# abhishekiitm/CSED_514_Project_Distributed_Training_using_PyTorch

Hardware: AMD Instinct MI355X
Metric: MNIST epoch time (s) + images/sec at 1/2/4/8 MI355X (DDP) (higher is better)
Workload: dtype bf16

## Files before the change

csrc/kernels/lenet_dev.h:

```cpp
#pragma once
#include <hip/hip_runtime.h>
#include <stdint.h>

#include "common.h"

namespace csed {

typedef short s16x8 __attribute__((ext_vector_type(8)));
typedef short s16x4 __attribute__((ext_vector_type(4)));
typedef unsigned short u16x4 __attribute__((ext_vector_type(4)));
typedef __attribute__((address_space(3))) s16x4 lds_s16x4;
typedef __attribute__((address_space(3))) void lds_void;
typedef __attribute__((address_space(1))) void glb_void;

template <typename T>
__device__ __forceinline__ unsigned short h16(float v) { return bits_of<T>((T)v); }
template <typename T>
__device__ __forceinline__ float f16v(unsigned short b) { return (float)of_bits<T>(b); }

__device__ __forceinline__ s16x4 lds_read_tr16(const unsigned short* p) {
  return __builtin_amdgcn_ds_read_tr16_b64_v4i16((lds_s16x4*)(p));
}


__device__ __forceinline__ int opaque(int x) {
  asm("" : "+v"(x));
  return x;
}

__device__ __forceinline__ void lds_barrier() { asm volatile("s_waitcnt lgkmcnt(0)\n\ts_barrier" ::: "memory"); }

template <int OFF>
__device__ __forceinline__ uint32_t lds_u16(const unsigned short* p) {
  uint32_t v;
  asm volatile("ds_read_u16 %0, %1 offset:%2" : "=v"(v) : "v"((uint32_t)reinterpret_cast<uintptr_t>(p)), "i"(OFF * 2));
  return v;
}
__device__ __forceinline__ void lds_wait8(uint32_t (&v)[8]) {
  asm volatile("s_waitcnt lgkmcnt(0)"
               : "+v"(v[0]), "+v"(v[1]), "+v"(v[2]), "+v"(v[3]), "+v"(v[4]), "+v"(v[5]), "+v"(v[6]), "+v"(v[7]));
}

__device__ __forceinline__ void store16_wt(const void* base, int byte_off, float4 v) {
  typedef unsigned int u32x4v_ __attribute__((ext_vector_type(4)));
  __builtin_amdgcn_raw_buffer_store_b128(__builtin_bit_cast(u32x4v_, v),
                                         __builtin_amdgcn_make_buffer_rsrc(const_cast<void*>(base), (short)0,
                                                                           0x7fffffff, 0x00020000),
                                         byte_off, 0, 16);
}

}
```

csrc/kernels/lenet_fused.hip:

```cpp
#include <algorithm>
#include <cmath>
#include <cstdlib>
#include <type_traits>

#include "comm/ipc_allreduce.h"
#include "common.h"
#include "dispatch.h"
#include "kernels/lenet_dev.h"
#include "kernels/lenet_images.h"
#include "kernels/lenet_layout.h"

namespace csed {

namespace lenet {
constexpr int LD_DC2 = 72, LD_DC1 = 592;
constexpr int LD_P1 = 148;
constexpr int NT = 1024, NW = 16;

constexpr int S_W2C = 0;
constexpr int S_W2D = (I_W2D - I_W2C) * 2;
constexpr int S_F1 = (I_F1 - I_W2C) * 2;
constexpr int WIMG_LDS_U4 = (I_END - I_W2C) / 8;
constexpr int S_X = (I_END - I_W2C) * 2;
constexpr int S_P1 = S_X + 800 * 2;
constexpr int S_I1 = S_P1 + 10 * LD_P1 * 2;
constexpr int S_P2 = S_I1 + (10 * LD_P1 + 15) / 16 * 16;
constexpr int S_I2 = S_P2 + 320 * 2;
constexpr int S_P1H = S_I2 + 320;
constexpr int S_DC2 = S_P1H + 12 * P1H_RP * 2;
constexpr int S_DC2H = S_DC2 + 32 * LD_DC2 * 2;
constexpr int S_DC1 = S_DC2H + 16 * DC2H_RP * 2;
constexpr int S_COFF = S_DC1 + 16 * LD_DC1 * 2;
constexpr int S_DOFF = S_COFF + 4 * 16 * 2;
constexpr int S_DZ1B = S_DOFF + 4 * 24 * 2;
constexpr int S_F = S_DZ1B + 64 * 2;
constexpr int F_D2S = 0, F_D1S = 32, F_H = 96, F_LOGIT = 160, F_PAR = 176, F_RED = 768, F_END = 2816;
constexpr int P_C1B = 0, P_C2B = 10, P_F1B = 30, P_F2B = 80, P_F2W = 90;
constexpr int S_W1C = S_F + F_END * 4;
constexpr int S_LABEL = S_W1C + 16 * 32 * 2;
constexpr int S_DBG = S_LABEL + 16;
constexpr int S_C1T = S_DBG + 32 * 8;
constexpr int S_C1H = S_C1T + 1024 * 8;
constexpr int S_XC = S_C1H + 1024 * 8;
constexpr int XC_LD = 800;
constexpr int S_CONSTB = S_XC + 3 * XC_LD * 2;
constexpr int S_TOTAL = S_CONSTB + 16 * 2;
static_assert(S_W2D % 16 == 0 && S_F1 % 16 == 0 && S_X % 16 == 0 && S_P1 % 16 == 0 && S_I1 % 16 == 0, "align");
static_assert(S_P2 % 16 == 0 && S_I2 % 16 == 0 && S_P1H % 16 == 0 && S_DC2 % 16 == 0 && S_DC2H % 16 == 0, "align");
static_assert(S_DC1 % 16 == 0 && S_COFF % 16 == 0 && S_DOFF % 16 == 0 && S_DZ1B % 16 == 0, "align");
static_assert(S_F % 16 == 0 && (F_RED * 4) % 16 == 0 && S_TOTAL <= 160 * 1024, "lds");
static_assert(WIMG_LDS_U4 % 256 == 0, "whole LDS-DMA rounds over waves 0-3");
static_assert(C2_KS * 32 <= LD_W2C && 25 * C2_ICP <= C2_KS * 32, "conv2 K");
static_assert(25 * DG_OCP <= DG_KS * 32, "dgrad K");
}

using namespace lenet;


constexpr int DBG_W = 32;
#define WSTAMP(w, i)                                                          \
  do {                                                                        \
    if (a.dbg && wave == (w) && lane == 0) DBGS[(i)] = __builtin_amdgcn_s_memtime(); \
  } while (0)
#define STAMP(i)                                                              \
  do {                                                                        \
    if (a.dbg && tid == 0 && s == (nsamp > 1 ? 1 : 0)) DBGS[(i)] = __builtin_amdgcn_s_memtime(); \
  } while (0)

__device__ const int64_t kZeroWord = 0;

__device__ __forceinline__ int64_t readlane64(int64_t v, int l) {
  const int lo = __builtin_amdgcn_readlane((int)(v & 0xffffffff), l);
  const int hi = __builtin_amdgcn_readlane((int)(v >> 32), l);
  return ((int64_t)hi << 32) | (uint32_t)lo;
}

template <typename T>
__device__ __forceinline__ void dgrad_store(unsigned short* DC1, int ci, int mm, float v, int bi) {
  const int ih = mm / 12, iw = mm - ih * 12;
  uint32_t* d = reinterpret_cast<uint32_t*>(DC1 + ci * LD_DC1 + (2 * ih) * 24 + 2 * iw);
  const uint32_t hv = h16<T>(v);
  d[0] = bi == 0 ? hv : (bi == 1 ? hv << 16 : 0u);
  d[12] = bi == 2 ? hv : (bi == 3 ? hv << 16 : 0u);
}

template <typename T>
__device__ __forceinline__ void dgrad_out(unsigned short* DC1, const unsigned short* P1, const uint8_t* I1,
                                          int ci, int mm, float v) {
  const int pi = ci * LD_P1 + mm;
  dgrad_store<T>(DC1, ci, mm, f16v<T>(P1[pi]) > 0.f ? v : 0.f, I1[pi]);
}

struct C1Tab {
  unsigned short v[NT][8];
};
constexpr C1Tab make_c1tab() {
  C1Tab t{};
  for (int tt = 0; tt < NT; ++tt) {
    const int tw = tt >> 6, tl16 = tt & 15, tkq = (tt & 63) >> 4;
    for (int it = 0; it < 3; ++it) {
      const int mt = (tw + it * NW) < 35 ? tw + it * NW : 35;
      const int m = mt * 16 + tl16;
      const int p = m >> 2, q = m & 3;
      t.v[tt][it] = (unsigned short)((2 * (p / 12) + (q >> 1)) * 28 + 2 * (p % 12) + (q & 1));
      const int w = mt * 4 + tkq;
      t.v[tt][4 + it] = (unsigned short)((w / 12) * P1H_RP + (w % 12) * LD_P1H);
    }
  }
  return t;
}
__constant__ C1Tab kC1Tab = make_c1tab();

constexpr int UP_C = 16, UP_S = 32, UP_MAXL = 8, UP_NT = UP_C * UP_S;

struct SplitNeed { uint32_t m[4]; };
__host__ __device__ constexpr SplitNeed split_need_table() {
  SplitNeed r{};
  for (int part = 0; part < 4; ++part) {
    uint32_t need = 0;
    for (int ts = 0; ts < (part == 0 ? 3 : 2); ++ts) {
      const int t = part + 4 * ts, py0 = (16 * t) / 12, py1 = (16 * t + 15) / 12;
      const int ps0 = (48 * py0) / 32, ps1 = (48 * (py1 + 1) - 1) / 32;
      need |= ((2u << ps1) - 1) & ~((1u << ps0) - 1);
    }
    r.m[part] = need;
  }
  return r;
}
__device__ constexpr SplitNeed kSplitNeed = split_need_table();

template <typename T, bool TRAIN, bool STAGED, int KS = 1>
__global__ void __launch_bounds__(NT, 1) lenet_train_kernel(LenetTrainArgs a, int write_logp, float* logp_out) {
  static_assert(KS == 1 || (KS == SPLIT_K && STAGED && TRAIN), "split step: staged training only");
  const uint64_t t_entry = __builtin_amdgcn_s_memtime();
  struct TrainKargs { LenetTrainArgs a; int write_logp; float* logp_out; };
// ... 78 lines not shown
  const bool stage_next = TRAIN && STAGED && a.stage_next;
  int64_t nrow = 0;
  uint32_t px_next = 0;
  int64_t lab_next = 0;
  auto conv1_tables = [&](int tt) {
    const int tw = tt >> 6, tl16 = tt & 15, tkq = (tt & 63) >> 4;
    u16x4 xo = {0, 0, 0, 0}, ho = {0, 0, 0, 0};
#pragma unroll
    for (int it = 0; it < 3; ++it) {
      const int mt = min(tw + it * NW, 35);
      const int m = mt * 16 + tl16;
      const int p = m >> 2, q = m & 3;
      xo[it] = (unsigned short)((2 * (p / 12) + (q >> 1)) * 28 + 2 * (p % 12) + (q & 1));
      const int w = mt * 4 + tkq;
      ho[it] = (unsigned short)((w / 12) * P1H_RP + (w % 12) * LD_P1H);
    }
    C1T[tt] = xo;
    C1H[tt] = ho;
  };
  if (wave < 4) {
    lds_barrier();
    constexpr int DMA_NT = 256;
    static_assert(WIMG_LDS_U4 % DMA_NT == 0, "whole LDS-DMA rounds over waves 0-3");
    const uint4* src = reinterpret_cast<const uint4*>(a.wimg + I_W2C);
#pragma unroll
    for (int u = 0; u < WIMG_LDS_U4 / DMA_NT; ++u)
      __builtin_amdgcn_global_load_lds((glb_void*)(const_cast<uint4*>(src + u * DMA_NT + tid)),
                                       (lds_void*)(wsm + S_W2C + (u * DMA_NT + wave * 64) * 16), 16, 0, 0);
    if (a.dbg && lane == 0) DBGS[(wave == 0 ? 10 : 17 + wave)] = __builtin_amdgcn_s_memtime();
  } else if (wave < 8) {
    const int t = tid - 256;
    if (a.dbg && t == 0) DBGS[17] = __builtin_amdgcn_s_memtime();
    int off0 = O_F2W - 90;
    off0 = t < 90 ? O_F2B - 80 : off0;
    off0 = t < 80 ? O_F1B - 30 : off0;
    off0 = t < 30 ? O_C2B - 10 : off0;
    off0 = t < 10 ? O_C1B : off0;
    float pv[3];
    pv[0] = a.params[off0 + t];
    pv[1] = a.params[O_F2W - 90 + 256 + t];
    pv[2] = a.params[O_F2W - 90 + min(512 + t, 589)];
    const uint4 w1 = reinterpret_cast<const uint4*>(a.wimg + I_W1C)[t & 63];
    uint32_t px0 = 0;
    int lab0 = 0;
    if (STAGED) {
      px0 = reinterpret_cast<const uint32_t*>(a.xstage + (int64_t)g * 784)[min(t, 195)];
      lab0 = (int)a.lstage[g];
    }
    if (KS == 1 && stage_next) {
      pbase = ((gptr64)curp)[opaque(0)] * (int64_t)a.B + b0;
      nrow = a.perm[min(pbase + a.B, a.perm_len - 1) + opaque(0)];
    }
    const uint64_t t_bar4 = __builtin_amdgcn_s_memtime();
    lds_barrier();
    if (t < 64) reinterpret_cast<uint4*>(W1Cs)[t] = w1;
#pragma unroll
    for (int j = 0; j < 3; ++j)
      if (t + j * 256 < 590) PAR[t + j * 256] = pv[j];
    if (STAGED) {
      if (t < 196) {
        u16x4 o;
#pragma unroll
        for (int j = 0; j < 4; ++j)
          o[j] = h16<T>(((float)((px0 >> (8 * j)) & 255u) * (1.f / 255.f) - a.mean) * inv_std);
        put_x(t, o);
      }
      if (t == 0) LABEL[0] = lab0;
    }
    if (a.dbg && t == 0) {
      DBGS[16] = __builtin_amdgcn_s_memtime();
      DBGS[15] = t_bar4;
    }
    asm volatile("" ::"v"(pv[0]), "v"(pv[1]), "v"(pv[2]), "v"(w1.x), "v"(w1.y), "v"(w1.z), "v"(w1.w), "v"(px0),
                 "v"(lab0));
  } else {
    int64_t cur = 0;
    if (STAGED) {
      rng_ctr = (uint64_t)((gptr64)rngp)[opaque(0)];
      if (KS > 1) cur = ((gptr64)curp)[opaque(0)];
    }
    const int t8 = tid - 512;
    const int tq = t8 < 64 ? t8 >> 4 : min(t8 - 64, 95) / 24;
    const int tks = t8 < 64 ? t8 & 15 : min(t8 - 64, 95) - 24 * tq;
    const int kg = t8 < 64 ? (int)kC2Order.fwd[min(4 * tks + tq, 49)] : (int)kDgOrder.fwd[min(4 * tks + tq, 74)];
    lds_barrier();
    if (t8 < 64) {
      const int tap = kg >> 1;
      COFF[t8] = (short)((tap / 5) * P1H_RP + (tap % 5) * LD_P1H + (kg & 1) * 8);
    } else if (t8 < 160) {
      const int tap = kg / 3, ocg = kg - 3 * tap;
      DOFF[t8 - 64] = (short)((tap / 5) * DC2H_RP + (tap % 5) * DG_OCP + ocg * 8);
    }
    if (!STAGED) {
      conv1_tables(tid - 512);
      conv1_tables(tid);
    }
    if (tid - 512 < 16) CONSTB[tid - 512] = tid - 512 < 8 ? (unsigned short)0 : h16<T>(1.f);
    if (STAGED) {
      if (KS > 1) pbase = cur * (int64_t)a.B + b0;
      const int tz = tid - 512;
      zero_p1h(tz);
      if (tz < 70) dropout_scales(tz, b0);
      asm volatile("" ::"v"(rng_ctr), "v"(pbase));
    }
  }
  if (!STAGED && nsamp > 0) {
    const int64_t row0 = perm_at(0);
    lab = (int)a.labels[row0];
    px = reinterpret_cast<const uint32_t*>(a.images + row0 * 784)[min(tid, 195)];
    rowv = perm_at(min(lane, nsamp - 1));
  }
  if (a.dbg && tid == 0) DBGS[13] = __builtin_amdgcn_s_memtime();
  int kwb[1];
  {
    const int k = min(wave * 16 + l16, 249), ic = k / 25, r = k % 25;
    kwb[0] = ic * LD_P1 + (r / 5) * 12 + (r % 5);
  }
  const int kc1 = (wave & 1) * 16 + l16;
  const int koffc1 = kc1 < 25 ? (kc1 / 5) * 28 + (kc1 % 5) : 0;

  f32x4 acc_c2[2][1];
#pragma unroll
  for (int i = 0; i < 2; ++i) acc_c2[i][0] = f32x4{0.f, 0.f, 0.f, 0.f};
  f32x4 acc_c1 = f32x4{0.f, 0.f, 0.f, 0.f};
  float loss_sum = 0.f, correct = 0.f;

  auto slab_at = [&](int e) { return a.slab + slab_off(slab_slot(e), e < O_C2W ? g : b0, G, R2); };
  float* SLF = reinterpret_cast<float*>(wsm + S_F1);
  static_assert(O_C2B + 20 <= (S_X - S_F1) / 4 && O_C2W % 4 == 0 && (O_C2B + 20) % 4 == 0, "conv2 row staging");
  auto stage_c2 = [&]() {
#pragma unroll
    for (int mt = 0; mt < 2; ++mt) {
      const int k = wave * 16 + l16;
#pragma unroll
      for (int r = 0; r < 4; ++r) {
        const int oc = mt * 16 + 4 * (lane >> 4) + r;
        if (oc < 20) {
          if (k <= 250) SLF[O_C2W + k * 20 + oc] = acc_c2[mt][0][r];
        }
      }
    }
  };
  auto store_c2 = [&](int t0, int nt) {
    for (int i = O_C2W / 4 + t0; i < (O_C2B + 20) / 4; i += nt)
      *reinterpret_cast<float4*>(a.slab + slab_off(S_C2 + 4 * i - O_C2W, b0, G, R2)) =
          reinterpret_cast<const float4*>(SLF)[i];
  };
  auto sample = [&](const int s, const int tid, const int lane, const int l16, const int kq, const int kb) {
    const int b = b0 + s * G;
    const bool wvec = TRAIN && own_vec;
    unsigned short* vs = TRAIN ? reinterpret_cast<unsigned short*>(a.vslab) + vec16_index(0, b) : nullptr;
    constexpr int vld = 4;
    if (a.dbg && lane == 0 && s == 0 && wave < 8) DBGS[24 + wave] = __builtin_amdgcn_s_memtime();
    lds_barrier();
    STAMP(0);
    if (KS > 1 && stage_next && wave >= 12 && s == 0) nrow = a.perm[min(pbase + a.B, a.perm_len - 1) + opaque(0)];
    if (!STAGED && wave >= 8) zero_p1h(tid - 512);
    const int t_lab = STAGED ? 0 : (s == 0 ? lab : __builtin_amdgcn_readlane(labv, s & 63));
    {
      if (tid < 196 && !STAGED) {
        u16x4 o;
#pragma unroll
        for (int j = 0; j < 4; ++j)
          o[j] = h16<T>(((float)((px >> (8 * j)) & 255u) * (1.f / 255.f) - a.mean) * inv_std);
        put_x(tid, o);
      }
      if (!STAGED && tid < 70) dropout_scales(tid, b);
      if (!STAGED && s + 1 < nsamp) {
        const int sn = s + 1;
        if ((sn & 63) == 0) rowv = perm_at(min(sn + lane, nsamp - 1));
        if (s == 0 || (sn & 63) == 0) labv = (int)a.labels[rowv];
        const int64_t rn = readlane64(rowv, sn & 63);
        px = reinterpret_cast<const uint32_t*>(a.images + rn * 784)[min(tid, 195)];
      }
    }
    if (!STAGED) lds_barrier();

    STAMP(1);
    {
      const u16x4 xo = STAGED ? __builtin_bit_cast(u16x4, make_uint2(c1row.x, c1row.y)) : C1T[tid];
      const u16x4 ho = STAGED ? __builtin_bit_cast(u16x4, make_uint2(c1row.z, c1row.w)) : C1H[tid];
      auto tiles = [&](auto nti) {
        constexpr int NTI = decltype(nti)::value;
        uint32_t rv[NTI][8];
#pragma unroll
        for (int it = 0; it < NTI; ++it) {
          const int pb = xo[it];
          const unsigned short* r1 = Xs + pb + 28 * kq;
          const unsigned short* r2 = Xs + pb + 112 + (kq == 1 ? W1_E1 : 0);
          rv[it][0] = lds_u16<0>(r1);
          rv[it][1] = lds_u16<1>(r1);
          rv[it][2] = lds_u16<2>(r1);
          rv[it][3] = lds_u16<3>(r1);
          rv[it][4] = lds_u16<4>(r1);
          rv[it][5] = lds_u16<0>(r2);
          rv[it][6] = lds_u16<1>(r2);
          rv[it][7] = lds_u16<2>(r2);
        }
        const float cb = PAR[P_C1B + min(l16, 9)];
        const frag fb1 = *reinterpret_cast<const frag*>(W1Cs + l16 * 32 + kb);
        f32x4 c[NTI];
#pragma unroll
        for (int it = 0; it < NTI; ++it) {
          lds_wait8(rv[it]);
          u16x8 raw;
#pragma unroll
          for (int j = 0; j < 8; ++j) raw[j] = (unsigned short)rv[it][j];
          c[it] = Mfma<T>::mma(__builtin_bit_cast(frag, raw), fb1, f32x4{0.f, 0.f, 0.f, 0.f});
        }
        if (l16 < 10) {
#pragma unroll
          for (int it = 0; it < NTI; ++it) {
            float best = c[it][0];
            int bi = 0;
#pragma unroll
            for (int r = 1; r < 4; ++r)
              if (c[it][r] > best) { best = c[it][r]; bi = r; }
            const int w = (wave + it * NW) * 4 + kq;
            const unsigned short hv = h16<T>(fmaxf(best + cb, 0.f));
            P1[l16 * LD_P1 + w] = hv;
            I1[l16 * LD_P1 + w] = (uint8_t)bi;
            P1H[ho[it] + l16] = hv;
          }
        }
      };
      static_assert(36 - 2 * NW == 4, "conv1: 3 tiles on waves 0-3, 2 on the rest");
      if (wave < 36 - 2 * NW) tiles(std::integral_constant<int, 3>{});
      else tiles(std::integral_constant<int, 2>{});
    }
    if (wave < 4) asm volatile("s_waitcnt vmcnt(0)" ::: "memory");
    if (a.dbg && tid == 0 && s == 0) DBGS[21] = __builtin_amdgcn_s_memtime();
    lds_barrier();

    STAMP(2);
    if (wave < 8) {
      const int mt = wave & 3, nt = wave >> 2;
      const int m = mt * 16 + l16;
      const int p = m >> 2, q = m & 3;
      const int oy = 2 * (p >> 2) + (q >> 1), ox = 2 * (p & 3) + (q & 1);
      const unsigned short* arow = P1H + oy * P1H_RP + ox * LD_P1H;
      const unsigned short* wrow = W2c + min(nt * 16 + l16, R_W2C) * LD_W2C + kb;
      const s16x8 co0 = *reinterpret_cast<const s16x8*>(COFF + kq * 16);
      const s16x8 co1 = *reinterpret_cast<const s16x8*>(COFF + kq * 16 + 8);
      f32x4 c0 = f32x4{0.f, 0.f, 0.f, 0.f}, c1 = c0;
#pragma unroll
      for (int ks = 0; ks < C2_KS; ++ks) {
        const frag fa = *reinterpret_cast<const frag*>(arow + (ks < 8 ? co0[ks] : co1[ks - 8]));
        const frag fb = *reinterpret_cast<const frag*>(wrow + ks * 32);
        if (ks & 1) c1 = Mfma<T>::mma(fa, fb, c1);
        else c0 = Mfma<T>::mma(fa, fb, c0);
      }
      const f32x4 c = c0 + c1;
      const int oc = nt * 16 + l16;
      if (oc < 20) {
        float best = c[0];
        int bi = 0;
#pragma unroll
        for (int r = 1; r < 4; ++r)
          if (c[r] > best) { best = c[r]; bi = r; }
        const int w = mt * 4 + kq;
        const unsigned short hv = h16<T>(fmaxf(best + PAR[P_C2B + oc], 0.f) * D2S[oc]);
        P2[oc * 16 + w] = hv;
        I2[oc * 16 + w] = (uint8_t)bi;
        if (wvec) vs[(V_P2 + oc * 16 + w) * vld] = hv;
      }
    }
    lds_barrier();

    STAMP(3);
    if (stage_next && (KS > 1 ? wave >= 12 : (wave >= 4 && wave < 8))) {
      px_next = reinterpret_cast<const uint32_t*>(a.images + nrow * 784)[min(tid & 255, 195)];
      lab_next = a.labels[nrow];
    }
    if (wave < 4) {
      const unsigned short* wrow = F1s + min(wave * 16 + l16, R_F1) * LD_F1 + kb;
      frag pa[10], fb[10];
#pragma unroll
      for (int ks = 0; ks < 10; ++ks) {
        pa[ks] = *reinterpret_cast<const frag*>(P2 + ks * 32 + kb);
        fb[ks] = *reinterpret_cast<const frag*>(wrow + ks * 32);
      }
      __builtin_amdgcn_sched_barrier(0);
      f32x4 c0 = f32x4{0.f, 0.f, 0.f, 0.f}, c1 = c0;
#pragma unroll
      for (int ks = 0; ks < 10; ++ks) {
        if (ks & 1) c1 = Mfma<T>::mma(pa[ks], fb[ks], c1);
        else c0 = Mfma<T>::mma(pa[ks], fb[ks], c0);
      }
      const f32x4 c = c0 + c1;
      if (lane < 16) {
        const int o = wave * 16 + lane;
        if (o < 50) {
          const float h = fmaxf(c[0] + PAR[P_F1B + o], 0.f) * D1S[o];
          Hs[o] = h;
          if (wvec) vs[(V_H + o) * vld] = h16<T>(h);
        }
      }
    }
    lds_barrier();

    STAMP(4);
    if (TRAIN && (wave & 3) != 0) {
      const int zt = (wave - 1 - (wave >> 2)) * 64 + lane;
      constexpr int ZN = 12 * 64;
      constexpr int NZ = (S_DC1 - S_DC2H) / 16;
      uint4* z = reinterpret_cast<uint4*>(DC2H);
      for (int i = zt; i < NZ; i += ZN) z[i] = make_uint4(0, 0, 0, 0);
      for (int m = zt; m < 784; m += ZN) {
        const unsigned short v = Xs[m];
#pragma unroll
        for (int k = 1; k < 4; ++k)
          if (m - k >= 0) XC[(k - 1) * XC_LD + m - k] = v;
      }
      if (KS > 1) {
        constexpr int NZ1 = (S_COFF - S_DC1) / 16;
        uint4* z1 = reinterpret_cast<uint4*>(DC1);
        for (int i = zt; i < NZ1; i += ZN) z1[i] = make_uint4(0, 0, 0, 0);
      }
    }
    if (wave == 0) {
      __builtin_amdgcn_s_setprio(3);
      const int t = STAGED ? LABEL[opaque(0)] : t_lab;
      const int o = min(lane, 49);
      float w2c[10];
#pragma unroll
      for (int c = 0; c < 10; ++c) w2c[c] = PAR[P_F2W + c * 50 + o];
      const float ho = Hs[o], d1 = D1S[o];
      const int c4 = min(lane >> 2, 9), q = lane & 3;
      const float* wr = PAR + P_F2W + c4 * 50;
      float zp0 = 0.f, zp1 = 0.f;
// ... 316 lines not shown
        if (ci < 10) {
          float v = 0.f;
  #pragma unroll
          for (int q = 0; q < 8; ++q) v += RED[q * 256 + rr * 16 + ci];
          dgrad_out<T>(DC1, P1, I1, ci, 128 + rr, v);
        }
      }
      lds_barrier();
  
    }

    STAMP(8);
    if (KS == 1 || wave < 12) {
      frag fa[3], fbv[3];
#pragma unroll
      for (int i = 0; i < 3; ++i) {
        const int ps = min((wave >> 1) + (KS > 1 ? 6 : 8) * i, 17);
        const int p0 = ps * 32 + kb;
        fa[i] = *reinterpret_cast<const frag*>(DC1 + l16 * LD_DC1 + p0);
        const int oh = p0 / 24, ow0 = p0 - oh * 24;
        const unsigned short* src = kc1 < 25 ? xrun(oh * 28 + ow0 + koffc1) : CONSTB + (kc1 == 25 ? 8 : 0);
        const uint2 lo = reinterpret_cast<const uint2*>(src)[0], hi = reinterpret_cast<const uint2*>(src)[1];
        fbv[i] = __builtin_bit_cast(frag, uint4{lo.x, lo.y, hi.x, hi.y});
      }
      const uint32_t need = KS > 1 ? kSplitNeed.m[part & 3] : (1u << 18) - 1;
#pragma unroll
      for (int i = 0; i < 3; ++i)
        if ((KS == 1 || wave < 12) && (wave >> 1) + (KS > 1 ? 6 : 8) * i < 18 &&
            ((need >> ((wave >> 1) + (KS > 1 ? 6 : 8) * i)) & 1u))
          acc_c1 = Mfma<T>::mma(fa[i], fbv[i], acc_c1);
    }
    STAMP(14);
  };
  for (int s = 0; s < nsamp; ++s) {
    const int t = opaque(tid);
    const int ln = t & 63;
    sample(s, t, ln, ln & 15, ln >> 4, 8 * (ln >> 4));
  }

  if (a.dbg && tid == 0) DBGS[11] = __builtin_amdgcn_s_memtime();
  if (TRAIN) {
    lds_barrier();
    auto part = [&](int w) { return w < 8 ? RED + w * 256 : reinterpret_cast<float*>(DC2H) + (w - 8) * 256; };
#pragma unroll
    for (int r = 0; r < 4; ++r) part(wave)[(4 * (lane >> 4) + r) * 16 + l16] = acc_c1[r];
    if (!STAGED) stage_c2();
    lds_barrier();
    if (tid < 512) {
      const int nt = tid >> 8, oc = (tid >> 4) & 15, col = tid & 15;
      float v = 0.f;
#pragma unroll
      for (int q = 0; q < 8; ++q) v += part(nt + 2 * q)[oc * 16 + col];
      const int k = nt * 16 + col;
      if (oc < 10) {
        if (k < 25) *slab_at(O_C1W + oc * 25 + k) = v;
        else if (k == 25) *slab_at(O_C1B + oc) = v;
      }
    } else if (!STAGED) {
      store_c2(tid - 512, NT - 512);
    }
  }
  if (tid == 0) {
    a.loss_acc[2 * g] = own_vec ? loss_sum : 0.f;
    a.loss_acc[2 * g + 1] = own_vec ? correct : 0.f;
  }
  if (a.dbg) {
    if (tid == 0) DBGS[23] = __builtin_amdgcn_s_memrealtime();
    __syncthreads();
    if (tid < DBG_W) a.dbg[g * DBG_W + tid] = DBGS[tid];
    if (a.dbg_entry && lane == 0) a.dbg_entry[g * NW + wave] = t_entry;
  }
}

#undef ACT

__device__ __forceinline__ void image_slots(int i, int& d0, int& d1) {
  d0 = d1 = -1;
  if (i < O_C1B) {
    d0 = I_W1C + (i / 25) * 32 + w1c_slot((i % 25) / 5, (i % 25) % 5);
  } else if (i >= O_C2W && i < O_C2B) {
    const int j = i - O_C2W;
    const int oc = j / 250, k = j % 250;
    const int ic = k / 25, r = k % 25, kh = r / 5, kw = r % 5;
    d0 = I_W2C + oc * LD_W2C + kC2Order.inv[r * 2 + (ic >> 3)] * 8 + (ic & 7);
    const int slice = kDgOrder.inv[((4 - kh) * 5 + (4 - kw)) * 3 + (oc >> 3)];
    d1 = I_W2D + (slice * 16 + ic) * 8 + (oc & 7);
  } else if (i >= O_F1W && i < O_F1B) {
    const int j = i - O_F1W;
    d0 = I_F1 + (j / 320) * LD_F1 + (j % 320);
  }
}

__device__ __forceinline__ void image_slots_flat(int i, int& d0, int& d1) {
  const int j = min(max(i - O_C2W, 0), O_C2B - O_C2W - 1);
  const int oc = j / 250, k = j % 250;
  const int ic = k / 25, r = k % 25, kh = r / 5, kw = r % 5;
  const int c2 = kC2Order.inv[r * 2 + (ic >> 3)];
  const int slice = kDgOrder.inv[((4 - kh) * 5 + (4 - kw)) * 3 + (oc >> 3)];
  const int i1 = min(max(i, 0), O_C1B - 1), r1 = i1 % 25;
  const int jf = min(max(i - O_F1W, 0), O_F1B - O_F1W - 1);
  const bool is_c1 = i < O_C1B, is_c2 = i >= O_C2W && i < O_C2B, is_f1 = i >= O_F1W && i < O_F1B;
  d0 = is_c1 ? I_W1C + (i1 / 25) * 32 + w1c_slot(r1 / 5, r1 % 5)
             : is_c2 ? I_W2C + oc * LD_W2C + c2 * 8 + (ic & 7) : is_f1 ? I_F1 + (jf / 320) * LD_F1 + (jf % 320) : -1;
  d1 = is_c2 ? I_W2D + (slice * 16 + ic) * 8 + (oc & 7) : -1;
}

template <typename T>
__device__ __forceinline__ float as_stored(float v) {
  if constexpr (!std::is_same<T, float>::value && !std::is_same<T, __bf16>::value) asm volatile("" : "+v"(v));
  return v;
}

template <typename T>
__device__ __forceinline__ void write_slots(unsigned short* wimg, int d0, int d1, float v) {
  if constexpr (!std::is_same<T, float>::value) {
    const unsigned short h = h16<T>(as_stored<T>(v));
    if (d0 >= 0) wimg[d0] = h;
    if (d1 >= 0) wimg[d1] = h;
  }
}

template <typename T>
__device__ __forceinline__ void write_images(unsigned short* wimg, int i, float v) {
  int d0, d1;
  image_slots(i, d0, d1);
  write_slots<T>(wimg, d0, d1, v);
}

template <typename T>
__global__ void lenet_pack_kernel(const float* __restrict__ params, unsigned short* __restrict__ wimg) {
  const int i = blockIdx.x * blockDim.x + threadIdx.x;
  if (i < NP) write_images<T>(wimg, i, params[i]);
}

static_assert(NB_CONV == N_CHUNKS, "one 64-slot slab chunk per CONV block half");
static_assert(UP_C * 4 == 64, "a CONV block half reduces one 64-slot slab chunk");
static_assert(UP_NT == 64 * UP_WAVES && SGD_BLOCKS == (NP + 255) / 256, "lenet_plan.h: update workgroup, SGD grid");
__host__ __device__ constexpr int fc_tile_of_block(int b) {
  const int q = (FC_TILES / 8) * (b % 8) + b / 8;
  return q < FC1_TILES ? (q % 4) * 21 + q / 4 : q;
}
__host__ __device__ constexpr bool fc_tile_map_is_bijective() {
  bool seen[FC_TILES] = {};
  for (int b = 0; b < FC_TILES; ++b) {
    const int t = fc_tile_of_block(b);
    if (t < 0 || t >= FC_TILES || seen[t]) return false;
    seen[t] = true;
  }
  return true;
}
static_assert(FC_TILES % 8 == 0 && fc_tile_map_is_bijective(), "FC tile map");

__device__ __forceinline__ void add4(float4& a, const float4& b) {
  a.x += b.x; a.y += b.y; a.z += b.z; a.w += b.w;
}

constexpr int STAGE_ROWS = 16;
constexpr int IMG_U4 = 784 / 16;

__device__ __forceinline__ void gather_batch(const LenetStageArgs& st, int64_t step, int64_t* rows_sh) {
  const int tid = threadIdx.x, nt = blockDim.x;
  const int r0 = blockIdx.x * STAGE_ROWS, nrows = min(STAGE_ROWS, st.rows - r0);
  for (int b = tid; b < nrows; b += nt) {
    const int64_t row = st.perm[min(step * st.B + (r0 + b) % st.B, st.perm_len - 1)];
    rows_sh[b] = row;
    st.lstage[r0 + b] = st.labels[row];
  }
  __syncthreads();
  const uint4* __restrict__ src = reinterpret_cast<const uint4*>(st.images);
  uint4* __restrict__ dst = reinterpret_cast<uint4*>(st.xstage) + (int64_t)r0 * IMG_U4;
  const int total = nrows * IMG_U4;
  constexpr int U = 8;
  for (int i0 = tid; i0 < total; i0 += nt * U) {
    uint4 v[U];
#pragma unroll
    for (int u = 0; u < U; ++u) {
      const int i = min(i0 + u * nt, total - 1);
      const int b = i / IMG_U4;
      v[u] = src[rows_sh[b] * IMG_U4 + (i - b * IMG_U4)];
    }
#pragma unroll
    for (int u = 0; u < U; ++u)
      if (i0 + u * nt < total) dst[i0 + u * nt] = v[u];
  }
}

// ... 1054 lines not shown
```

csrc/kernels/lenet_images.h:

```cpp
#pragma once
#include <hip/hip_runtime.h>
#include <stdint.h>

namespace csed {
namespace lenet {

constexpr int C2_ICP = 16;
constexpr int LD_P1H = 24;
constexpr int C2_KS = 13;
constexpr int P1H_RP = 320;
constexpr int DG_OCP = 24;
constexpr int DG_KS = 19;
constexpr int DC2H_RP = 16 * 24 + 32;
struct DgOrder {
  uint8_t fwd[75], inv[75];
};
struct C2Order {
  uint8_t fwd[50], inv[50];
};
constexpr C2Order make_c2_order() {
  C2Order o{{42, 2, 43, 41, 27, 37, 26, 31, 5, 1, 29, 19, 34, 24, 33, 18, 48, 13, 14, 16, 12, 10, 38, 28, 23,
             3, 22, 32, 17, 47, 39, 49, 20, 30, 35, 15, 8, 6, 21, 46, 36, 11, 4, 0, 25, 45, 7, 9, 44, 40},
            {}};
  for (int i = 0; i < 50; ++i) o.inv[o.fwd[i]] = (uint8_t)i;
  return o;
}
constexpr bool c2_order_is_permutation() {
  const C2Order o = make_c2_order();
  for (int c = 0; c < 50; ++c)
    if (o.fwd[o.inv[c]] != c) return false;
  return true;
}
static_assert(c2_order_is_permutation(), "C2_ORDER must be a permutation of the 50 K slices");
static __constant__ C2Order kC2Order = make_c2_order();
constexpr DgOrder make_dg_order() {
  DgOrder o{{10, 70, 33, 22, 35, 46, 63, 52, 49, 27, 66, 6, 7, 56, 11, 71, 64, 53, 47, 74, 36, 42, 51, 40, 16,
             54, 68, 57, 65, 5, 24, 21, 45, 12, 67, 18, 55, 17, 50, 1, 28, 19, 9, 58, 60, 0, 20, 29, 59, 32,
             13, 73, 38, 44, 61, 39, 8, 30, 41, 3, 14, 25, 69, 31, 23, 72, 4, 15, 62, 2, 26, 48, 43, 34, 37},
            {}};
  for (int i = 0; i < 75; ++i) o.inv[o.fwd[i]] = (uint8_t)i;
  return o;
}
constexpr bool dg_order_is_permutation() {
  const DgOrder o = make_dg_order();
  for (int c = 0; c < 75; ++c)
    if (o.fwd[o.inv[c]] != c) return false;
  return true;
}
static_assert(dg_order_is_permutation(), "DG_ORDER must be a permutation of the 75 K slices");
static __constant__ DgOrder kDgOrder = make_dg_order();
constexpr int LD_W2C = 432, LD_F1 = 328;
constexpr int R_W2C = 20, R_F1 = 50;
constexpr int DG_CH = 4 * DG_KS + 1;
constexpr int I_W1C = 0, I_W2C = 512;
constexpr int w1c_slot(int kh, int kw) {
  return kh < 4 ? kh * 8 + kw : (kw < 2 ? 5 + kw : 8 + 5 + (kw - 2));
}
constexpr int W1_E1 = 2;
constexpr int I_W2D = I_W2C + (R_W2C + 1) * LD_W2C;
constexpr int I_F1 = I_W2D + DG_CH * 16 * 8;
constexpr int I_END = I_W2C + ((I_F1 + (R_F1 + 1) * LD_F1 - I_W2C + 4095) / 4096) * 4096;

}
}
```

csrc/kernels/lenet_tile.hip:

```cpp
#include <algorithm>
#include <type_traits>

#include "common.h"
#include "dispatch.h"
#include "kernels/lenet_dev.h"
#include "kernels/lenet_images.h"
#include "kernels/lenet_layout.h"
#include "launchers.h"

namespace csed {
namespace lenet_tile {

using namespace csed::lenet;
constexpr int TS = kLenetTileSamples;
constexpr int NT = 1024, NW = 16;
constexpr int X_LD = 804;
constexpr int XCP = TS * X_LD + 32;
constexpr int P1H_SZ = 12 * P1H_RP;
constexpr int DC2_LD = 80, DC2_SZ = 20 * DC2_LD + 24;
constexpr int DCH_SZ = 64 * DG_OCP + 120;
constexpr int I1_LD = 148, I1_SZ = 10 * I1_LD;
constexpr int F_D2S = 0, F_D1S = TS * 20, F_H = F_D1S + TS * 52, F_LAB = F_H + TS * 64, F_LOSS = F_LAB + TS,
              F_END = (F_LOSS + 2 * TS + 3) / 4 * 4;
constexpr int D_W1C = 0;
// ... 48 lines not shown
  unsigned short* X = reinterpret_cast<unsigned short*>(dsm + D_X);
  unsigned short* P1H = reinterpret_cast<unsigned short*>(dsm + D_P1H);
  uint8_t* I1 = dsm + D_I1;
  unsigned short* P2 = reinterpret_cast<unsigned short*>(dsm + D_P2);
  uint8_t* I2 = dsm + D_I2;
  float* Fs = reinterpret_cast<float*>(dsm + D_F);
  float* const MSK_D2S[2] = {Fs + F_D2S, reinterpret_cast<float*>(dsm + D_MSK)};
  float* const MSK_D1S[2] = {Fs + F_D1S, reinterpret_cast<float*>(dsm + D_MSK) + TS * 20};
  float* Hs = Fs + F_H;
  int* LAB = reinterpret_cast<int*>(Fs + F_LAB);
  float* LOSS = Fs + F_LOSS;
  unsigned short* DZ1B = reinterpret_cast<unsigned short*>(dsm + D_DZ1B);
  unsigned short* DC2 = reinterpret_cast<unsigned short*>(dsm + D_DC2);
  unsigned short* DCH = reinterpret_cast<unsigned short*>(dsm + D_DCH);
  auto DY1 = [&](int s) {
    return reinterpret_cast<unsigned short*>(dsm + (s < 2 ? D_P1H : D_DC2)) + (s & 1) * DY1_SZ;
  };
  uint64_t* DBGS = reinterpret_cast<uint64_t*>(dsm + D_DBG);
#define TSTAMP(i)                                                                   \
  do {                                                                              \
    if (a.dbg && tid == 0 && tile == g) DBGS[(i)] = __builtin_amdgcn_s_memtime(); \
  } while (0)
  if (a.dbg && threadIdx.x == 0) {
    DBGS[0] = __builtin_amdgcn_s_memtime();
    DBGS[12] = __builtin_amdgcn_s_memrealtime();
  }

  const int tid = threadIdx.x, lane = tid & 63;
  const int wave = __builtin_amdgcn_readfirstlane(tid >> 6);
  const int l16 = lane & 15, kq = lane >> 4, kb = 8 * kq;
  const int G = a.grid, g = blockIdx.x, B = a.B;
  const int ntile = (B + TS - 1) / TS;
  unsigned short* const VH = reinterpret_cast<unsigned short*>(a.vslab);
  const float inv_std = 1.f / a.std_;
  const int lane0 = opaque(0);
  const int64_t cur0 = (a.cursor ? a.cursor : &kTileZero)[lane0];
  const uint64_t rng_ctr = (uint64_t)((TRAIN && a.rng_offset) ? a.rng_offset : &kTileZero)[lane0];
  const int64_t pbase = cur0 * (int64_t)B;
  auto perm_at = [&](int b) { return a.perm[min(pbase + (int64_t)min(b, B - 1), a.perm_len - 1)]; };
  const unsigned short one = h16<T>(1.f);
  auto draw_masks = [&](int tl, int par, int t) {
    if (t < TS * 70) {
      const int s = t / 70, u = t - 70 * s;
      float sc = 1.f;
      if (TRAIN) {
        uint32_t k0 = (uint32_t)a.seed, k1 = (uint32_t)(a.seed >> 32);
        asm volatile("" : "+s"(k0), "+s"(k1));
        const uint64_t e = (uint64_t)(a.rank_stride * (int64_t)B + tl * TS + s) * 70ull + u;
        sc = dropout_keep(((uint64_t)k1 << 32) | k0, rng_ctr << 20, e, a.drop_p) ? 1.f / (1.f - a.drop_p) : 0.f;
      }
      if (u < 20) MSK_D2S[par][s * 20 + u] = sc;
      else MSK_D1S[par][s * 52 + u - 20] = sc;
    }
  };
  const int s_me = min(tid / 196, TS - 1), q_me = tid - 196 * (tid / 196);
  const bool px_thread = tid < TS * 196;
  uint32_t px = 0, px_next = 0;
  int lab = 0;
  int64_t nrow = 0, srow = 0, lab_next = 0;
  const bool staged = a.xstage != nullptr;
  const bool stage_next = TRAIN && staged && a.stage_next;
  if (staged && px_thread && g < ntile) {
    px = reinterpret_cast<const uint32_t*>(a.xstage + (int64_t)(g * TS + s_me) * 784)[q_me];
    if (q_me == 0) lab = reinterpret_cast<const int*>(a.lstage + g * TS + s_me)[0];
  }

  if (wave < 4) {
    const uint4* src = reinterpret_cast<const uint4*>(a.wimg + I_W2C);
#pragma unroll
    for (int u = 0; u < W_BYTES / 16 / 256; ++u)
      __builtin_amdgcn_global_load_lds((glb_void*)(const_cast<uint4*>(src + u * 256 + tid)),
                                       (lds_void*)(wsm + (u * 256 + wave * 64) * 16), 16, 0, 0);
    asm volatile("s_waitcnt vmcnt(0)" ::: "memory");
  } else if (wave < 8) {
    const int t = tid - 256;
    auto par_index = [](int q) {
      return q < 10 ? O_C1B + q : q < 30 ? O_C2B + q - 10 : q < 80 ? O_F1B + q - 30 : q < 90 ? O_F2B + q - 80
                                                                                          : O_F2W + q - 90;
    };
    float pv[3];
#pragma unroll
    for (int j = 0; j < 3; ++j) pv[j] = a.params[par_index(min(t + j * 256, 589))];
    const uint4 w1c = reinterpret_cast<const uint4*>(a.wimg + I_W1C)[min(t, 63)];
    const int tq = (t >> 4) & 3, tks = t & 15;
    const int kg2 = (int)kC2Order.fwd[min(4 * tks + tq, 49)];
    const int jd = min(max(t - 64, 0), 79), qd = jd / 20, ksd = jd - 20 * qd;
    const int kgd = (int)kDgOrder.fwd[min(4 * min(ksd, DG_KS - 1) + qd, 74)];
#pragma unroll
    for (int j = 0; j < 3; ++j)
      if (t + j * 256 < 590) PAR[t + j * 256] = pv[j];
    if (t < 64) {
      reinterpret_cast<uint4*>(W1Cs)[t] = w1c;
      const int tap = kg2 >> 1;
      COFF[t] = (short)((tap / 5) * P1H_RP + (tap % 5) * LD_P1H + (kg2 & 1) * 8);
    } else if (t < 64 + 80) {
      const int tap = kgd / 3, ocg = kgd - 3 * tap, ty = tap / 5, tx = tap % 5;
      DGT[jd] = ((ty * 8 + tx) * DG_OCP + ocg * 8) | (tap << 16);
    } else if (t < 64 + 80 + 48) {
      const int j = t - 144;
      const unsigned short o = h16<T>(1.f);
      reinterpret_cast<u16x8*>(dsm + D_ONES)[j] = j < 24 ? u16x8{o, o, o, o, o, o, o, o} : u16x8{0, 0, 0, 0, 0, 0, 0, 0};
    }
  } else {
    const int t = tid - 512;
    uint4* z = reinterpret_cast<uint4*>(P1H);
    for (int i = t; i < TS * P1H_SZ * 2 / 16; i += 512) z[i] = make_uint4(0, 0, 0, 0);
    uint4* zh = reinterpret_cast<uint4*>(DCH);
    for (int i = t; i < TS * DCH_SZ * 2 / 16; i += 512) zh[i] = make_uint4(0, 0, 0, 0);
    if (g < ntile) draw_masks(g, 0, t);
  }
  if (!staged && px_thread && g < ntile) {
    const int64_t row = perm_at(g * TS + s_me);
    px = reinterpret_cast<const uint32_t*>(a.images + row * 784)[q_me];
    if (q_me == 0) lab = (int)a.labels[row];
  }
  __syncthreads();
  if (a.dbg && threadIdx.x == 0) DBGS[1] = __builtin_amdgcn_s_memtime();

  f32x4 acc_w[2][2];
#pragma unroll
  for (int t = 0; t < 2; ++t) acc_w[t][0] = acc_w[t][1] = f32x4{0.f, 0.f, 0.f, 0.f};
  f32x4 acc_c1 = f32x4{0.f, 0.f, 0.f, 0.f};
  float loss_sum = 0.f, correct = 0.f;
  auto pool4 = [](const f32x4& c, float& best, int& bi) {
    best = c[0];
    bi = 0;
#pragma unroll
    for (int r = 1; r < 4; ++r)
      if (c[r] > best) { best = c[r]; bi = r; }
  };

  const int wave_o = wave;
  for (int tile = g; tile < ntile; tile += G) {
    const int tid = opaque(threadIdx.x), lane = tid & 63, l16 = lane & 15, kq = lane >> 4, kb = 8 * kq;
    const int wave = ONE_TILE ? __builtin_amdgcn_readfirstlane(tid >> 6) : wave_o;
    const int s_me = min(tid / 196, TS - 1), q_me = tid - 196 * (tid / 196);
    const int b0 = tile * TS;
    const int par = ((tile - g) / G) & 1;
    float* const D2S = MSK_D2S[par];
    float* const D1S = MSK_D1S[par];
    TSTAMP(2);
    if (px_thread) {
      const bool ok = b0 + s_me < B;
      u16x4 o;
#pragma unroll
      for (int j = 0; j < 4; ++j)
        o[j] = ok ? h16<T>(((float)((px >> (8 * j)) & 255u) * (1.f / 255.f) - a.mean) * inv_std) : (unsigned short)0;
      *reinterpret_cast<u16x4*>(X + s_me * X_LD + 4 * q_me) = o;
      unsigned short* x1 = X + XCP + s_me * X_LD + 4 * q_me - 1;
      if (q_me > 0) x1[0] = o[0];
      *reinterpret_cast<uint32_t*>(x1 + 1) = o[1] | ((uint32_t)o[2] << 16);
      x1[3] = o[3];
      if (q_me == 0) LAB[s_me] = lab;
    }
    if (a.dbg && tid == 0 && tile == g) DBGS[14] = __builtin_amdgcn_s_memtime();
    if (tile == g) {
      if (stage_next && px_thread)
        srow = a.perm[min((cur0 + 1) * (int64_t)B + min(g * TS + s_me, B - 1), a.perm_len - 1)];
      if (px_thread && g + G < ntile) nrow = perm_at((g + G) * TS + s_me);
    }
    if (a.dbg && lane == 0 && tile == g) DBGS[16 + wave] = __builtin_amdgcn_s_memtime();
    lds_barrier();

    TSTAMP(3);
    {
      const int wsmp = wave >> 2, wq = wave & 3;
      const frag fb1 = *reinterpret_cast<const frag*>(W1Cs + l16 * 32 + kb);
      const float cb = PAR[P_C1B + min(l16, 9)];
      const int q1 = l16 & 3;
      const int xl = (q1 >> 1) * 28 + 2 * (l16 >> 2) + (q1 & 1);
      const int o1 = xl + 28 * kq, o2 = xl + 112 + (kq == 1 ? W1_E1 : 0);
      const uint32_t* xr1 = reinterpret_cast<const uint32_t*>(X + (o1 & 1) * XCP + (o1 & ~1));
      const unsigned short* xe1 = X + o1 + 4;
      const uint32_t* xr2 = reinterpret_cast<const uint32_t*>(X + (o2 & 1) * XCP + (o2 & ~1));
      const unsigned short* xe2 = X + o2 + 2;
      const int pl = kq * LD_P1H + min(l16, 9), il = min(l16, 9) * I1_LD + kq;
#pragma unroll
      for (int grp = 0; grp < 3; ++grp) {
        uint32_t r0[3], r1[3], e4[3], r2[3], e2[3];
#pragma unroll
        for (int it = 0; it < 3; ++it) {
          const int k = 3 * grp + it;
          const int xs = wsmp * X_LD + wq * 168 + (k / 3) * 56 + 8 * (k % 3);
          r0[it] = xr1[xs / 2];
          r1[it] = xr1[xs / 2 + 1];
          e4[it] = xe1[xs];
          r2[it] = xr2[xs / 2];
          e2[it] = xe2[xs];
        }
#pragma unroll
        for (int it = 0; it < 3; ++it) {
          const uint4 raw = make_uint4(r0[it], r1[it], e4[it] | (r2[it] << 16), (r2[it] >> 16) | (e2[it] << 16));
          const f32x4 c = Mfma<T>::mma(__builtin_bit_cast(frag, raw), fb1, f32x4{0.f, 0.f, 0.f, 0.f});
          const int k = 3 * grp + it, mt3 = 3 * wq + k / 3, mtr = k % 3;
          float best;
          int bi;
          pool4(c, best, bi);
          if (l16 < 10) {
            const unsigned short hv = h16<T>(fmaxf(best + cb, 0.f));
            P1H[wsmp * P1H_SZ + mt3 * P1H_RP + (4 * mtr) * LD_P1H + pl] = hv;
            I1[wsmp * I1_SZ + 4 * (3 * mt3 + mtr) + il] = (uint8_t)((hv & 0x7fff) ? bi : 4);
          }
        }
      }
    }
    lds_barrier();

    TSTAMP(4);
    {
      const int s = wave >> 2, mt = wave & 3;
      const int m = mt * 16 + l16, p = m >> 2, q = m & 3;
      const int oy = 2 * (p >> 2) + (q >> 1), ox = 2 * (p & 3) + (q & 1);
      const unsigned short* arow = P1H + s * P1H_SZ + oy * P1H_RP + ox * LD_P1H;
      const unsigned short* w0 = W2c + min(l16, R_W2C) * LD_W2C + kb;
      const unsigned short* w1 = W2c + min(16 + l16, R_W2C) * LD_W2C + kb;
      const s16x8 co0 = *reinterpret_cast<const s16x8*>(COFF + kq * 16);
      const s16x8 co1 = *reinterpret_cast<const s16x8*>(COFF + kq * 16 + 8);
      f32x4 c0 = f32x4{0.f, 0.f, 0.f, 0.f}, c1 = c0, e0 = c0, e1 = c0;
#pragma unroll
      for (int ks = 0; ks < C2_KS; ++ks) {
        const frag fa = *reinterpret_cast<const frag*>(arow + (ks < 8 ? co0[ks] : co1[ks - 8]));
        const frag fb0 = *reinterpret_cast<const frag*>(w0 + ks * 32);
        const frag fb1 = *reinterpret_cast<const frag*>(w1 + ks * 32);
        if (ks & 1) {
          e0 = Mfma<T>::mma(fa, fb0, e0);
          e1 = Mfma<T>::mma(fa, fb1, e1);
        } else {
          c0 = Mfma<T>::mma(fa, fb0, c0);
          c1 = Mfma<T>::mma(fa, fb1, c1);
        }
      }
      c0 += e0;
      c1 += e1;
      const int b = b0 + s;
      const int w = mt * 4 + kq;
#pragma unroll
      for (int nt = 0; nt < 2; ++nt) {
        const int oc = nt * 16 + l16;
        if (oc < 20) {
          float best;
          int bi;
          pool4(nt ? c1 : c0, best, bi);
          const unsigned short hv = h16<T>(fmaxf(best + PAR[P_C2B + oc], 0.f) * D2S[s * 20 + oc]);
          P2[s * 320 + oc * 16 + w] = hv;
          I2[s * 320 + oc * 16 + w] = (uint8_t)bi;
          if (TRAIN && b < B) VH[vec16_index(V_P2 + oc * 16 + w, b)] = hv;
        }
      }
    }
    lds_barrier();

    TSTAMP(5);
    if (wave < 4) {
      const unsigned short* wrow = F1s + min(wave * 16 + l16, R_F1) * LD_F1 + kb;
      const unsigned short* prow = P2 + (l16 >> 2) * 320 + kb;
      f32x4 c0 = f32x4{0.f, 0.f, 0.f, 0.f}, c1 = c0;
#pragma unroll
      for (int ks = 0; ks < 10; ++ks) {
        const frag pa = *reinterpret_cast<const frag*>(prow + ks * 32);
        const frag fb = *reinterpret_cast<const frag*>(wrow + ks * 32);
        if (ks & 1) c1 = Mfma<T>::mma(pa, fb, c1);
        else c0 = Mfma<T>::mma(pa, fb, c0);
      }
      const float cz = c0[0] + c1[0];
      const int o = wave * 16 + l16;
      if (o < 50) {
        const float h = fmaxf(cz + PAR[P_F1B + o], 0.f) * D1S[kq * 52 + o];
        Hs[kq * 64 + o] = h;
        if (TRAIN && b0 + kq < B) VH[vec16_index(V_H + o, b0 + kq)] = h16<T>(h);
      }
    }
    lds_barrier();

    TSTAMP(6);
    if (wave >= TS && tile + G < ntile) draw_masks(tile + G, par ^ 1, tid - 64 * TS);
    if (wave < TS) {
      const int s = wave, b = b0 + s;
      const bool valid = b < B;
      const int t = LAB[s + opaque(0)];
      const float* H = Hs + s * 64;
      const int o = min(lane, 49);
      float w2c[10];
#pragma unroll
      for (int c = 0; c < 10; ++c) w2c[c] = PAR[P_F2W + c * 50 + o];
      const float ho = H[o], d1 = D1S[s * 52 + o];
      const int c4 = min(lane >> 2, 9), q = lane & 3;
      const float* wr = PAR + P_F2W + c4 * 50;
      float zp0 = 0.f, zp1 = 0.f;
#pragma unroll
      for (int u = 0; u < 13; ++u) {
        const int oo = q * 13 + u, oc = min(oo, 49);
        const float wv = oo < 50 ? wr[oc] : 0.f;
        if (u & 1) zp1 = fmaf(wv, H[oc], zp1);
        else zp0 = fmaf(wv, H[oc], zp0);
      }
      float zp = zp0 + zp1;
      zp += __builtin_bit_cast(float, __builtin_amdgcn_update_dpp(0, __builtin_bit_cast(int, zp), 0xB1, 0xf, 0xf,
                                                                   false));
      zp += __builtin_bit_cast(float, __builtin_amdgcn_update_dpp(0, __builtin_bit_cast(int, zp), 0x4E, 0xf, 0xf,
                                                                   false));
      const float w2t = PAR[P_F2W + t * 50 + o];
      float lg[10];
#pragma unroll
      for (int c = 0; c < 10; ++c)
// ... 330 lines not shown
```

Measured before the change: 4.758 million.

## Repack conv2 K dimension to drop channel padding, using gathered pair loads

Conv2's GEMM K layout is repacked. Previously 10 input channels were padded to 16 per tap, giving 13 MFMA k-steps. Now the first 8 channels of each tap use dense 8-wide fragment loads, and the remaining 2 channels of each tap are packed four taps per fragment via 32-bit gathers, cutting K to 8 k-steps and shrinking the weight row stride. The goal is fewer MFMAs and less weight traffic, at the cost of four scalar LDS reads per gathered fragment in the last two k-steps.

```diff
diff --git a/csrc/kernels/lenet_dev.h b/csrc/kernels/lenet_dev.h
--- a/csrc/kernels/lenet_dev.h
+++ b/csrc/kernels/lenet_dev.h
@@ -20,6 +20,15 @@
 
 __device__ __forceinline__ s16x4 lds_read_tr16(const unsigned short* p) {
   return __builtin_amdgcn_ds_read_tr16_b64_v4i16((lds_s16x4*)(p));
+}
+
+template <typename F>
+__device__ __forceinline__ F c2_gather(const unsigned short* a, const s16x8& off, int j) {
+  typedef uint32_t u32x4v_ __attribute__((ext_vector_type(4)));
+  u32x4v_ v;
+#pragma unroll
+  for (int p = 0; p < 4; ++p) v[p] = *reinterpret_cast<const uint32_t*>(a + off[j + p]);
+  return __builtin_bit_cast(F, v);
 }
 
 
diff --git a/csrc/kernels/lenet_fused.hip b/csrc/kernels/lenet_fused.hip
--- a/csrc/kernels/lenet_fused.hip
+++ b/csrc/kernels/lenet_fused.hip
@@ -50,7 +50,7 @@
 static_assert(S_DC1 % 16 == 0 && S_COFF % 16 == 0 && S_DOFF % 16 == 0 && S_DZ1B % 16 == 0, "align");
 static_assert(S_F % 16 == 0 && (F_RED * 4) % 16 == 0 && S_TOTAL <= 160 * 1024, "lds");
 static_assert(WIMG_LDS_U4 % 256 == 0, "whole LDS-DMA rounds over waves 0-3");
-static_assert(C2_KS * 32 <= LD_W2C && 25 * C2_ICP <= C2_KS * 32, "conv2 K");
+static_assert(C2_KS * 32 <= LD_W2C && 25 * 10 <= C2_KS * 32 && 4 * C2_DKS + 8 == 4 * C2_KS, "conv2 K");
 static_assert(25 * DG_OCP <= DG_KS * 32, "dgrad K");
 }
 
@@ -295,11 +295,10 @@
     const int t8 = tid - 512;
     const int tq = t8 < 64 ? t8 >> 4 : min(t8 - 64, 95) / 24;
     const int tks = t8 < 64 ? t8 & 15 : min(t8 - 64, 95) - 24 * tq;
-    const int kg = t8 < 64 ? (int)kC2Order.fwd[min(4 * tks + tq, 49)] : (int)kDgOrder.fwd[min(4 * tks + tq, 74)];
+    const int kg = t8 < 64 ? (int)kC2Pack.coff[max(t8, 0)] : (int)kDgOrder.fwd[min(4 * tks + tq, 74)];
     lds_barrier();
     if (t8 < 64) {
-      const int tap = kg >> 1;
-      COFF[t8] = (short)((tap / 5) * P1H_RP + (tap % 5) * LD_P1H + (kg & 1) * 8);
+      COFF[t8] = (short)kg;
     } else if (t8 < 160) {
       const int tap = kg / 3, ocg = kg - 3 * tap;
       DOFF[t8 - 64] = (short)((tap / 5) * DC2H_RP + (tap % 5) * DG_OCP + ocg * 8);
@@ -458,7 +457,8 @@
       f32x4 c0 = f32x4{0.f, 0.f, 0.f, 0.f}, c1 = c0;
 #pragma unroll
       for (int ks = 0; ks < C2_KS; ++ks) {
-        const frag fa = *reinterpret_cast<const frag*>(arow + (ks < 8 ? co0[ks] : co1[ks - 8]));
+        const frag fa = ks < C2_DKS ? *reinterpret_cast<const frag*>(arow + co0[ks])
+                                    : c2_gather<frag>(arow, co1, 4 * (ks - C2_DKS));
         const frag fb = *reinterpret_cast<const frag*>(wrow + ks * 32);
         if (ks & 1) c1 = Mfma<T>::mma(fa, fb, c1);
         else c0 = Mfma<T>::mma(fa, fb, c0);
@@ -941,7 +941,7 @@
     const int j = i - O_C2W;
     const int oc = j / 250, k = j % 250;
     const int ic = k / 25, r = k % 25, kh = r / 5, kw = r % 5;
-    d0 = I_W2C + oc * LD_W2C + kC2Order.inv[r * 2 + (ic >> 3)] * 8 + (ic & 7);
+    d0 = I_W2C + oc * LD_W2C + c2_col(kC2Pack, ic, r);
     const int slice = kDgOrder.inv[((4 - kh) * 5 + (4 - kw)) * 3 + (oc >> 3)];
     d1 = I_W2D + (slice * 16 + ic) * 8 + (oc & 7);
   } else if (i >= O_F1W && i < O_F1B) {
@@ -954,13 +954,13 @@
   const int j = min(max(i - O_C2W, 0), O_C2B - O_C2W - 1);
   const int oc = j / 250, k = j % 250;
   const int ic = k / 25, r = k % 25, kh = r / 5, kw = r % 5;
-  const int c2 = kC2Order.inv[r * 2 + (ic >> 3)];
+  const int c2 = c2_col(kC2Pack, ic, r);
   const int slice = kDgOrder.inv[((4 - kh) * 5 + (4 - kw)) * 3 + (oc >> 3)];
   const int i1 = min(max(i, 0), O_C1B - 1), r1 = i1 % 25;
   const int jf = min(max(i - O_F1W, 0), O_F1B - O_F1W - 1);
   const bool is_c1 = i < O_C1B, is_c2 = i >= O_C2W && i < O_C2B, is_f1 = i >= O_F1W && i < O_F1B;
   d0 = is_c1 ? I_W1C + (i1 / 25) * 32 + w1c_slot(r1 / 5, r1 % 5)
-             : is_c2 ? I_W2C + oc * LD_W2C + c2 * 8 + (ic & 7) : is_f1 ? I_F1 + (jf / 320) * LD_F1 + (jf % 320) : -1;
+             : is_c2 ? I_W2C + oc * LD_W2C + c2 : is_f1 ? I_F1 + (jf / 320) * LD_F1 + (jf % 320) : -1;
   d1 = is_c2 ? I_W2D + (slice * 16 + ic) * 8 + (oc & 7) : -1;
 }
 
diff --git a/csrc/kernels/lenet_images.h b/csrc/kernels/lenet_images.h
--- a/csrc/kernels/lenet_images.h
+++ b/csrc/kernels/lenet_images.h
@@ -5,9 +5,9 @@
 namespace csed {
 namespace lenet {
 
-constexpr int C2_ICP = 16;
 constexpr int LD_P1H = 24;
-constexpr int C2_KS = 13;
+constexpr int C2_KS = 8;
+constexpr int C2_DKS = 6;
 constexpr int P1H_RP = 320;
 constexpr int DG_OCP = 24;
 constexpr int DG_KS = 19;
@@ -15,24 +15,44 @@
 struct DgOrder {
   uint8_t fwd[75], inv[75];
 };
-struct C2Order {
-  uint8_t fwd[50], inv[50];
+struct C2Pack {
+  uint8_t dense[25];
+  uint8_t pair[25];
+  short coff[64];
+  bool ok;
 };
-constexpr C2Order make_c2_order() {
-  C2Order o{{42, 2, 43, 41, 27, 37, 26, 31, 5, 1, 29, 19, 34, 24, 33, 18, 48, 13, 14, 16, 12, 10, 38, 28, 23,
-             3, 22, 32, 17, 47, 39, 49, 20, 30, 35, 15, 8, 6, 21, 46, 36, 11, 4, 0, 25, 45, 7, 9, 44, 40},
-            {}};
-  for (int i = 0; i < 50; ++i) o.inv[o.fwd[i]] = (uint8_t)i;
-  return o;
+constexpr int c2_tap_off(int tap) { return (tap / 5) * P1H_RP + (tap % 5) * LD_P1H; }
+constexpr C2Pack make_c2_pack() {
+  constexpr int C2_DENSE[25] = {4,  24, 23, 18, 17, 22, 0, 2, 5, 10, 11, 13, 20,
+                                21, 1,  3,  19, 14, 8,  6, 7, 12, 15, 16, 9};
+  constexpr int C2_PAIR[7][4] = {{-1, 14, 1, 12}, {16, 0, 15, 3}, {21, 5, 20, 8}, {17, 7, 24, 4},
+                                 {22, 2, 19, 9},  {6, 23, -1, 18}, {11, -1, 10, 13}};
+  C2Pack t{};
+  int nd[25] = {}, np[25] = {};
+  for (int s = 0; s < 25; ++s) {
+    t.dense[C2_DENSE[s]] = (uint8_t)s;
+    ++nd[C2_DENSE[s]];
+    if (s < 4 * C2_DKS) t.coff[(s & 3) * 16 + (s >> 2)] = (short)c2_tap_off(C2_DENSE[s]);
+  }
+  for (int pc = 0; pc < 4; ++pc) t.coff[8 + pc] = (short)(c2_tap_off(C2_DENSE[24]) + 2 * pc);
+  for (int i = 0; i < 7; ++i)
+    for (int pc = 0; pc < 4; ++pc) {
+      const int s = 25 + i, tap = C2_PAIR[i][pc];
+      t.coff[(s & 3) * 16 + 8 + 4 * ((s >> 2) - C2_DKS) + pc] = (short)(tap < 0 ? 10 : c2_tap_off(tap) + 8);
+      if (tap >= 0) {
+        t.pair[tap] = (uint8_t)(4 * s + pc);
+        ++np[tap];
+      }
+    }
+  t.ok = true;
+  for (int tap = 0; tap < 25; ++tap) t.ok = t.ok && nd[tap] == 1 && np[tap] == 1;
+  return t;
 }
-constexpr bool c2_order_is_permutation() {
-  const C2Order o = make_c2_order();
-  for (int c = 0; c < 50; ++c)
-    if (o.fwd[o.inv[c]] != c) return false;
-  return true;
+static_assert(make_c2_pack().ok, "C2_DENSE / C2_PAIR must place every (tap, channel) of conv2 exactly once");
+static __constant__ C2Pack kC2Pack = make_c2_pack();
+__host__ __device__ constexpr int c2_col(const C2Pack& t, int ic, int tap) {
+  return ic < 8 ? t.dense[tap] * 8 + ic : t.pair[tap] * 2 + (ic - 8);
 }
-static_assert(c2_order_is_permutation(), "C2_ORDER must be a permutation of the 50 K slices");
-static __constant__ C2Order kC2Order = make_c2_order();
 constexpr DgOrder make_dg_order() {
   DgOrder o{{10, 70, 33, 22, 35, 46, 63, 52, 49, 27, 66, 6, 7, 56, 11, 71, 64, 53, 47, 74, 36, 42, 51, 40, 16,
              54, 68, 57, 65, 5, 24, 21, 45, 12, 67, 18, 55, 17, 50, 1, 28, 19, 9, 58, 60, 0, 20, 29, 59, 32,
@@ -49,7 +69,7 @@
 }
 static_assert(dg_order_is_permutation(), "DG_ORDER must be a permutation of the 75 K slices");
 static __constant__ DgOrder kDgOrder = make_dg_order();
-constexpr int LD_W2C = 432, LD_F1 = 328;
+constexpr int LD_W2C = 272, LD_F1 = 328;
 constexpr int R_W2C = 20, R_F1 = 50;
 constexpr int DG_CH = 4 * DG_KS + 1;
 constexpr int I_W1C = 0, I_W2C = 512;
diff --git a/csrc/kernels/lenet_tile.hip b/csrc/kernels/lenet_tile.hip
--- a/csrc/kernels/lenet_tile.hip
+++ b/csrc/kernels/lenet_tile.hip
@@ -154,8 +154,7 @@
 #pragma unroll
     for (int j = 0; j < 3; ++j) pv[j] = a.params[par_index(min(t + j * 256, 589))];
     const uint4 w1c = reinterpret_cast<const uint4*>(a.wimg + I_W1C)[min(t, 63)];
-    const int tq = (t >> 4) & 3, tks = t & 15;
-    const int kg2 = (int)kC2Order.fwd[min(4 * tks + tq, 49)];
+    const int kg2 = (int)kC2Pack.coff[t & 63];
     const int jd = min(max(t - 64, 0), 79), qd = jd / 20, ksd = jd - 20 * qd;
     const int kgd = (int)kDgOrder.fwd[min(4 * min(ksd, DG_KS - 1) + qd, 74)];
 #pragma unroll
@@ -163,8 +162,7 @@
       if (t + j * 256 < 590) PAR[t + j * 256] = pv[j];
     if (t < 64) {
       reinterpret_cast<uint4*>(W1Cs)[t] = w1c;
-      const int tap = kg2 >> 1;
-      COFF[t] = (short)((tap / 5) * P1H_RP + (tap % 5) * LD_P1H + (kg2 & 1) * 8);
+      COFF[t] = (short)kg2;
     } else if (t < 64 + 80) {
       const int tap = kgd / 3, ocg = kgd - 3 * tap, ty = tap / 5, tx = tap % 5;
       DGT[jd] = ((ty * 8 + tx) * DG_OCP + ocg * 8) | (tap << 16);
@@ -291,7 +289,8 @@
       f32x4 c0 = f32x4{0.f, 0.f, 0.f, 0.f}, c1 = c0, e0 = c0, e1 = c0;
 #pragma unroll
       for (int ks = 0; ks < C2_KS; ++ks) {
-        const frag fa = *reinterpret_cast<const frag*>(arow + (ks < 8 ? co0[ks] : co1[ks - 8]));
+        const frag fa = ks < C2_DKS ? *reinterpret_cast<const frag*>(arow + co0[ks])
+                                    : c2_gather<frag>(arow, co1, 4 * (ks - C2_DKS));
         const frag fb0 = *reinterpret_cast<const frag*>(w0 + ks * 32);
         const frag fb1 = *reinterpret_cast<const frag*>(w1 + ks * 32);
         if (ks & 1) {
```

Result: no change. 4.786 million, median of 6 (+0.6%).
